# url-kaist/UV-SLAM

Hardware: AMD Instinct MI355X
Metric: sliding-window solves/sec (10 KF, 150 pts, 40 lines, 3 VP) (higher is better)
Workload: dtype f64; 1 GPU; W10-P150-L40-V3 x 256 independent windows per GPU (BASELINE configs[2]); single window (configs[1]) in single_window, the 20k-point window (configs[3]) in large_window (both with --full); windows_per_gpu=256, frames=11, points=150, lines=40, vp_tagged_lines=30, prior=True, parallelism=replicas x1

## Files before the change

uv-slam_amd/csrc/uvs_solve_kernel.h:

```cpp
#pragma once
#include <hip/hip_runtime.h>
#include <utility>
#include "../../include/uvs_solver.h"
#include "uvs_layout.h"
#include "uvs_factors.h"

namespace uvsdev {


#ifndef UVS_X_PLAIN_TID
static __device__ __forceinline__ int lane_tid() { int t = threadIdx.x; asm volatile("" : "+v"(t)); return t; }
#else
static __device__ __forceinline__ int lane_tid() { return threadIdx.x; }
#endif
static constexpr int NT = UVS_NT;
static constexpr int NW = NT / 64;
static constexpr bool ROLES = NT > 256;
static constexpr int ET = ROLES ? 256 : NT;
static constexpr int EW = ET / 64;
static constexpr int GT0 = NT - UVS_GT;
UVS_DEV int wave_uniform() { return __builtin_amdgcn_readfirstlane((int)(threadIdx.x >> 6)); }
UVS_DEV bool role_eval() { return !ROLES || wave_uniform() < EW; }
#ifndef UVS_X_NO_LINE_ROTATE
UVS_DEV int line_lane() { return ROLES ? (lane_tid() ^ 256) : lane_tid(); }
// ... 101 lines not shown
    *sq = g; *rsq = 2.0 * hh;
}
UVS_DEV void block_reduce(double* sh, double* s , double* mx) {
    const int tid = lane_tid(), lane = tid & 63, wv = tid >> 6;
    __syncthreads();
#pragma unroll
    for (int k = 0; k < 4; ++k) { const double t = wave_sum(s[k]); if (lane == 0) sh[L_RED + wv * 5 + k] = t; }
    { const double t = wave_max(*mx); if (lane == 0) sh[L_RED + wv * 5 + 4] = t; }
    __syncthreads();
    double a[4] = {0, 0, 0, 0}, m = 0.0;
#pragma unroll
    for (int w = 0; w < NW; ++w) {
#pragma unroll
        for (int k = 0; k < 4; ++k) a[k] += sh[L_RED + w * 5 + k];
        m = fmax(m, sh[L_RED + w * 5 + 4]);
    }
#pragma unroll
    for (int k = 0; k < 4; ++k) s[k] = a[k];
    *mx = m;
}

UVS_DEV void lacc_set(double* sh, double cost, double gmax) {
    const int tid = lane_tid();
    if (tid < ET) sh[L_LCOST + tid] = cost;
    const double wm = wave_max(gmax);
    if ((tid & 63) == 0) sh[L_LGMAX + (tid >> 6)] = wm;
}
UVS_DEV void lacc_add(double* sh, double cost, double gmax) {
    const int tid = lane_tid();
    if (tid < ET) sh[L_LCOST + tid] += cost;
    const double wm = wave_max(gmax);
    if ((tid & 63) == 0) sh[L_LGMAX + (tid >> 6)] = fmax(sh[L_LGMAX + (tid >> 6)], wm);
}
UVS_DEV double lacc_cost(const double* sh) { const int tid = lane_tid(); return tid < ET ? sh[L_LCOST + tid] : 0.0; }
UVS_DEV double lacc_gmax(const double* sh) { return sh[L_LGMAX + (lane_tid() >> 6)]; }

struct Ctx {
    const DevWin* hdr;
    const double* bd;
    const int* bi;
    double* ws;
    double* sh;
    KOpts o;
    int ltrig_ok = 0;
    int ptab_ok = 0;
};

UVS_DEV const double* line_trig_of(const Ctx& c, const double* line) {
    const DevWin& h = *c.hdr;
    if (!c.ltrig_ok) return nullptr;
    return line == c.ws + h.w_line0 ? c.ws + h.w_ltrig0 : (line == c.ws + h.w_line1 ? c.ws + h.w_ltrig1 : nullptr);
}

UVS_DEV void stage_rotations(const Ctx& c, const double* x) {
    const int tid = lane_tid();
    if (tid < UVS_NF) quat_to_R(x + 7 * tid + 3, c.sh + L_RF + 9 * tid);
    else if (tid == UVS_NF) { quat_to_R(x + 176 + 3, c.sh + L_EX); c.sh[L_EX + 9] = x[176]; c.sh[L_EX + 10] = x[177]; c.sh[L_EX + 11] = x[178]; }
    else if (tid == UVS_RELO_FRAME && c.hdr->relo_on) quat_to_R(x + 184 + 3, c.sh + L_RF + 9 * UVS_RELO_FRAME);
}
UVS_DEV const double* pose_of(const double* x, int f) { return x + (f > UVS_NF ? 184 : 7 * f); }

UVS_DEV void load_point_obs(const Ctx& c, int o, double td, double* pi, double* pj, double* vij) {
    const DevWin& h = *c.hdr;
    const double* m = c.bd + h.d_ptmeas + o; const int st = h.pt_stride;
    pi[0] = m[0]; pi[1] = m[st]; pi[2] = m[2 * st]; pj[0] = m[3 * st]; pj[1] = m[4 * st]; pj[2] = m[5 * st];
    if (h.td_on) {
        const double* v = c.bd + h.d_ptvel + o;
        vij[0] = v[0]; vij[1] = v[st]; vij[2] = v[2 * st]; vij[3] = v[3 * st];
        const double di = td - v[4 * st], dj = td - v[5 * st];
        pi[0] -= di * vij[0]; pi[1] -= di * vij[1]; pj[0] -= dj * vij[2]; pj[1] -= dj * vij[3];
    }
}

UVS_DEV void stage_prior_tables(const Ctx& c) {
    const int tid = lane_tid();
    const DevWin& h = *c.hdr;
    if (h.prior_n <= 0) return;
    int* tab = (int*)(c.sh + L_PTAB);
    if (tid < 4 * UVS_MAX_PRIOR_BLOCKS) tab[tid] = c.bi[h.i_prior + tid];
    if (tid < 9 * UVS_MAX_PRIOR_BLOCKS) c.sh[L_PX0 + tid] = c.bd[h.d_prior + h.prior_n * h.prior_n + 2 * h.prior_n + tid];
}
UVS_DEV void prior_dx(const Ctx& c, const double* x) {
    const int tid = lane_tid() - 64;
    const DevWin& h = *c.hdr;
    if (h.prior_n > 0 && tid >= 0 && tid < h.prior_nb) {
        int kind, frame, size, idx;
        double x0[9];
        if (c.ptab_ok) {
            const int* tab = (const int*)(c.sh + L_PTAB);
            kind = tab[tid]; frame = tab[16 + tid]; size = tab[32 + tid]; idx = tab[48 + tid];
#pragma unroll
            for (int k = 0; k < 9; ++k) x0[k] = c.sh[L_PX0 + 9 * tid + k];
        } else {
            const int* pt = c.bi + h.i_prior;
            kind = pt[tid]; frame = pt[16 + tid]; size = pt[32 + tid]; idx = pt[48 + tid];
            const double* x0g = c.bd + h.d_prior + h.prior_n * h.prior_n + 2 * h.prior_n + 9 * tid;
#pragma unroll
            for (int k = 0; k < 9; ++k) x0[k] = x0g[k];
        }
        const double* xb = (kind == UVS_BLOCK_POSE) ? x + 7 * frame : (kind == UVS_BLOCK_SPEEDBIAS) ? x + 77 + 9 * frame : (kind == UVS_BLOCK_TD) ? x + 183 : x + 176;
        double* dx = c.sh + L_PDX + idx;
        if (size != 7) { for (int k = 0; k < size; ++k) dx[k] = xb[k] - x0[k]; }
        else {
            dx[0] = xb[0] - x0[0]; dx[1] = xb[1] - x0[1]; dx[2] = xb[2] - x0[2];
            double qi[4], e[4]; quat_inv(x0 + 3, qi); quat_mul(qi, xb + 3, e);
            const double sg = (e[3] >= 0.0) ? 2.0 : -2.0;
            dx[3] = sg * e[0]; dx[4] = sg * e[1]; dx[5] = sg * e[2];
        }
    }
}
UVS_DEV double prior_quad(const Ctx& c, int dst = L_PR) {
    const DevWin& h = *c.hdr;
    const int n = h.prior_n, tid = lane_tid();
    double cost = 0.0;
    if (n <= 0) return cost;
    const double* H0 = c.ws + h.w_prior_h0;
    const int parts = (NT / n) < 4 ? (NT / n) : 4;
    const int part = tid / n, row = tid - part * n;
    const double g0v = tid < n ? c.ws[h.w_prior_h0 + UVS_PH_G0(n) + tid] : 0.0, c0v = tid == 0 ? c.ws[h.w_prior_h0 + UVS_PH_C0(n)] : 0.0;
    if (part < parts) {
        const int kb = (n * part) / parts, ke = (n * (part + 1)) / parts;
        double p8[8] = {0, 0, 0, 0, 0, 0, 0, 0};
        for (int k = kb; k < ke; k += PR_UN) {
            double jv[PR_UN];
#pragma unroll
            for (int u = 0; u < PR_UN; ++u) jv[u] = H0[(k + u < ke ? k + u : kb) * n + row];
#pragma unroll
            for (int u = 0; u < PR_UN; ++u) if (k + u < ke) p8[u & 7] += jv[u] * c.sh[L_PDX + k + u];
        }
        c.sh[L_S + 128 * part + row] = ((p8[0] + p8[1]) + (p8[2] + p8[3])) + ((p8[4] + p8[5]) + (p8[6] + p8[7]));
    }
    __syncthreads();
    if (tid < n) {
        double y = c.sh[L_S + tid];
        for (int p = 1; p < parts; ++p) y += c.sh[L_S + 128 * p + tid];
        c.sh[dst + tid] = y;
        cost = c.sh[L_PDX + tid] * (g0v + 0.5 * y);
        if (tid == 0) cost += c0v;
    }
    return cost;
}
UVS_DEV double prior_cost_share(const Ctx& c, int src) {
    const DevWin& h = *c.hdr;
    const int n = h.prior_n, tid = lane_tid();
    double cost = 0.0;
    if (tid < n) {
        cost = c.sh[L_PDX + tid] * (c.ws[h.w_prior_h0 + UVS_PH_G0(n) + tid] + 0.5 * c.sh[src + tid]);
        if (tid == 0) cost += c.ws[h.w_prior_h0 + UVS_PH_C0(n)];
    }
    return cost;
}
UVS_DEV double prior_residual_rows(const Ctx& c) {
    const DevWin& h = *c.hdr;
    const int n = h.prior_n, tid = lane_tid();
    double cost = 0.0;
    if (tid < n) {
        const double* Jr = c.bd + h.d_prior + (size_t)tid * n;
        double s = c.bd[h.d_prior + n * n + tid];
        for (int k = 0; k < n; ++k) s += Jr[k] * c.sh[L_PDX + k];
        c.sh[L_PR + tid] = s;
        cost = 0.5 * s * s;
    }
    return cost;
}

UVS_DEV void cost_imu_raw(const Ctx& c, const double* x, int lane0) {
    const DevWin& h = *c.hdr;
    const int b = lane_tid() - lane0;
    double* rs = c.sh + L_S + 1024;
    if (b >= 0 && b < h.n_imu) {
        const int fi = c.bi[h.i_imu + 2 * b], skip = c.bi[h.i_imu + 2 * b + 1];
        if (!skip) {
            const double* blk = c.bd + h.d_imu + (size_t)b * UVS_IMU_STRIDE;
            double r[15];
            imu_raw(blk, blk + UVS_IMU_JAC, c.o.G, x + 7 * fi, x + 77 + 9 * fi, x + 7 * (fi + 1), x + 77 + 9 * (fi + 1), r, nullptr);
#pragma unroll
            for (int i = 0; i < 15; ++i) rs[16 * b + i] = r[i];
        }
    }
}
template <int PB = CP_PB, int LB = CP_LB>
UVS_DEV double cost_pass(const Ctx& c, const double* x, const double* invd, const double* line, int po0, int po1, int lo0, int lo1, bool with_imu) {
    const DevWin& h = *c.hdr;
    const int tid = lane_tid();
    const double* RF = c.sh + L_RF; const double* ric = c.sh + L_EX; const double* tic = c.sh + L_EX + 9;
    const double* ltrig = line_trig_of(c, line);
    double cost = 0.0;
    long long tq_ = clock64();
#define UVS_CQ(slot) if (c.o.debug == 1 && tid == 0) { const long long t_ = clock64(); c.sh[L_WPROF + slot] += (double)(t_ - tq_); tq_ = t_; }
    const int imu_lane0 = ROLES ? NT - 64 : 0;
#ifndef UVS_X_NO_IMU_WAVE
    if (ROLES && with_imu) cost_imu_raw(c, x, imu_lane0);
#endif
    for (int o0 = po0 + tid; o0 < po1; o0 += PB * NT) {
        int lm[PB], fi[PB], fj[PB]; bool in[PB];
        double pi[PB][3], pj[PB][3], vij[PB][4], idp[PB];
#pragma unroll
        for (int u = 0; u < PB; ++u) {
            const int o = o0 + u * NT; in[u] = o < po1;
            const int oo = in[u] ? o : o0;
            lm[u] = c.bi[h.i_pt_lm + oo]; fi[u] = c.bi[h.i_pt_fi + oo]; fj[u] = c.bi[h.i_pt_fj + oo];
            load_point_obs(c, oo, x[183], pi[u], pj[u], vij[u]);
        }
#pragma unroll
        for (int u = 0; u < PB; ++u) idp[u] = invd[lm[u]];
#pragma unroll
        for (int u = 0; u < PB; ++u) {
            if (!in[u]) continue;
            double r[2];
            point_eval<false, false>(x + 7 * fi[u], RF + 9 * fi[u], pose_of(x, fj[u]), RF + 9 * fj[u], ric, tic, idp[u], pi[u], pj[u], c.o.sqrt_info, r, nullptr, nullptr, nullptr, nullptr);
            double sc; cost += 0.5 * cauchy(c.o.loss_pt, r[0] * r[0] + r[1] * r[1], &sc);
        }
    }
    for (int o0 = lo0 + UVS_COST_LINE_LANE; o0 < lo1; o0 += LB * NT) {
        int lm[LB], fj[LB], hv[LB]; bool in[LB];
        double ms[LB][9], lp[LB][4] = {}, tg[LB][8];
        const int st = h.ln_stride;
#pragma unroll
        for (int u = 0; u < LB; ++u) {
            const int o = o0 + u * NT; in[u] = o < lo1;
            const int oo = in[u] ? o : o0;
            lm[u] = c.bi[h.i_ln_lm + oo]; fj[u] = c.bi[h.i_ln_fj + oo]; hv[u] = c.bi[h.i_ln_vp + oo];
            const double* m = c.bd + h.d_lnmeas + oo;
#pragma unroll
            for (int q = 0; q < 9; ++q) ms[u][q] = m[q * st];
        }
#pragma unroll
        for (int u = 0; u < LB; ++u) {
            if (ltrig) {
#pragma unroll
                for (int q = 0; q < 8; ++q) tg[u][q] = ltrig[8 * lm[u] + q];
            } else {
#pragma unroll
                for (int q = 0; q < 4; ++q) lp[u][q] = line[4 * lm[u] + q];
            }
        }
#pragma unroll
        for (int u = 0; u < LB; ++u) {
            if (!in[u]) continue;
            const double sp[3] = {ms[u][0], ms[u][1], ms[u][2]}, ep[3] = {ms[u][3], ms[u][4], ms[u][5]}, vp[3] = {ms[u][6], ms[u][7], ms[u][8]};
            LineGeom g;
            line_geom<false>(x + 7 * fj[u], x + 7 * fj[u] + 3, RF + 9 * fj[u], ric, tic, lp[u], g, ltrig ? tg[u] : nullptr);
            double r[2], sc;
            line_residual<false>(g, sp, ep, c.o.line_factor, r, nullptr, nullptr);
            cost += 0.5 * cauchy(c.o.loss_ln, r[0] * r[0] + r[1] * r[1], &sc);
            if (hv[u]) { double rv; vp_residual<false>(g, vp, c.o.vp_factor, &rv, nullptr, nullptr); cost += 0.5 * cauchy(c.o.loss_vp, rv * rv, &sc); }
        }
    }
    UVS_CQ(2)
    if (with_imu) {
        double* rs = c.sh + L_S + 1024;
#ifndef UVS_X_NO_IMU_WAVE
        if (!ROLES)
#endif
        cost_imu_raw(c, x, 0);
        __syncthreads();
        const int b = tid >> 4, i = tid & 15;
        if (b < h.n_imu && i < 15 && !c.bi[h.i_imu + 2 * b + 1]) {
            const double* W = c.ws + h.w_imu_w + (size_t)b * UVS_IMU_WS + i * 15;
            double wv[15];
#pragma unroll
            for (int k = 0; k < 15; ++k) wv[k] = (k >= i) ? W[k] : 0.0;
            double sacc = 0.0;
#pragma unroll
            for (int k = 0; k < 15; ++k) sacc += wv[k] * rs[16 * b + k];
            cost += 0.5 * sacc * sacc;
        }
    }
    UVS_CQ(3)
    return cost;
}

typedef double d4_t __attribute__((ext_vector_type(4)));

UVS_DEV double* sblk(double* sh, int i, int j) { return sh + L_S + (((i * (i + 1)) >> 1) + j) * UVS_BLK_SZ; }

UVS_DEV double rcp_newton(double x) {
    double y = __builtin_amdgcn_rcp(x);
    double e = fma(-x, y, 1.0); y = fma(y, e, y);
    e = fma(-x, y, 1.0); y = fma(y, e, y);
    return y;
}

struct MiniCtx { double* sh; struct { int debug; } o; };
template <bool TR = false>
UVS_DEV void chol_update_item(double* sh, int i, int cc, int j0, int j1, int lane, d4_t& acc) {
    const int li = lane & 15, lk = lane >> 4;
    const bool rhs = (i == UVS_NF);
    const double* Bj = sblk(sh, cc, j0) + li * UVS_BLK_LD + lk;
    const double* Ai = rhs ? sh + L_DLT + 16 * j0 + lk : sblk(sh, i, j0) + li * UVS_BLK_LD + lk;
    const int astep = rhs ? 16 : UVS_BLK_SZ;
    if (j0 >= j1) return;
    double a0[4], b0[4], a1[4], b1[4];
#define UVS_CH_LOAD(AV, BV) { _Pragma("unroll") for (int q = 0; q < 4; ++q) { AV[q] = Ai[4 * q]; BV[q] = Bj[4 * q]; } Bj += UVS_BLK_SZ; Ai += astep; }
#define UVS_CH_MFMA(AV, BV) { _Pragma("unroll") for (int q = 0; q < 4; ++q) acc = TR ? __builtin_amdgcn_mfma_f64_16x16x4f64(BV[q], AV[q], acc, 0, 0, 1) : __builtin_amdgcn_mfma_f64_16x16x4f64(AV[q], BV[q], acc, 0, 0, 1); }
    UVS_CH_LOAD(a0, b0)
    for (int j = j0;;) {
        if (j + 1 < j1) UVS_CH_LOAD(a1, b1)
        UVS_CH_MFMA(a0, b0)
        if (++j >= j1) break;
        if (j + 1 < j1) UVS_CH_LOAD(a0, b0)
        UVS_CH_MFMA(a1, b1)
        if (++j >= j1) break;
    }
// ... 1843 lines not shown
        asm_imu(c, N);
    }
#ifndef UVS_X_NO_PRIOR_AHEAD
    asm_prior_add(c, pa);
#else
    asm_prior(c);
#endif
    __syncthreads();
    UVS_TLOG(c, 26);
    asm_finish(c, x, first && !redamp, radius, lacc_cost(c.sh) + ic, lacc_gmax(c.sh), 0);
    UVS_TLOG(c, 27);
}

UVS_DEV void linearize(const Ctx& c, const double* x, const double* invd, const double* line, bool first, double radius, int prep_mode, GAcc& A) {
    if (ROLES) { linearize_roles(c, x, invd, line, first, radius, prep_mode, false); return; }
    const DevWin& h = *c.hdr;
    const int grp = gather_group(c);
    gacc_zero(A);
    { const double pc = lin_prep(c, x, prep_mode); lacc_set(c.sh, pc, 0.0); }
    {
        ChunkDesc d = chunk_desc(c, 0);
        for (int ch = 0; ch < h.n_chunks; ++ch) {
            chunk_eval(c, d, x, invd, line, first, radius);
            chunk_gather(c, d, grp, A);
            if (ch + 1 < h.n_chunks) d = chunk_desc(c, ch + 1);
        }
    }
    ImuN N;
    const double ic = lin_imu(c, x, N);
    lin_assemble(c, x, first, radius, grp, A, N, lacc_cost(c.sh) + ic, lacc_gmax(c.sh));
}

UVS_DEV void relinearize_damping(const Ctx& c, const double* x, double radius, GAcc& A) {
    if (ROLES) { linearize_roles(c, x, nullptr, nullptr, false, radius, 2, true); return; }
    const DevWin& h = *c.hdr;
    const int grp = gather_group(c);
    (void)lin_prep(c, x, 2);
    {
        ChunkDesc d = chunk_desc(c, 0);
        for (int ch = 0; ch < h.n_chunks; ++ch) {
            redamp_prep(c, d, radius);
            redamp_gather(c, d, grp, A);
            if (ch + 1 < h.n_chunks) d = chunk_desc(c, ch + 1);
        }
    }
    ImuN N;
    const double ic = lin_imu(c, x, N);
    lin_assemble(c, x, false, radius, grp, A, N, lacc_cost(c.sh) + ic, lacc_gmax(c.sh));
}

#ifndef UVS_BS_FRAME_LANE0
#define UVS_BS_FRAME_LANE0 192
#endif
template <int LNBT = BS_LNB, int PSB = 4, bool STREAM = false>
UVS_DEV void backsub_candidate(const Ctx& c, const double* invd, const double* line, double* invd_c, double* line_c,
                                  int pk0, int pk1, int lk0, int lk1, bool with_frames, double* sums_out, double* lstep = nullptr) {
    const DevWin& h = *c.hdr;
    double* sh = c.sh;
    const int tid = lane_tid();
    const double* d = sh + L_DLT;
    double gd = 0.0, dd2 = 0.0, step2 = 0.0, xc2 = 0.0;
    const bool td_on = h.td_on != 0;
    const bool ex_on = h.ex_on != 0, relo_on = h.relo_on != 0;
    double* ltrig_c = const_cast<double*>(line_trig_of(c, line_c));
    const bool relo2 = h.relo2 != 0;
    if (relo2) relo2_backsub(c);
    else if (relo_on) {
        if (tid < 6) sh[L_DLT + 16 * UVS_RELO_FRAME + tid] = d[UVS_EX_INDEX(tid)];
        __syncthreads();
    }
    if (with_frames && tid < UVS_RD && ((tid & 15) < 15 || (td_on && tid == UVS_TD_INDEX) || ((ex_on | relo_on) && tid < 96))) { gd += sh[L_G + tid] * d[tid]; dd2 += sh[L_DD + tid] * d[tid] * d[tid]; }
    const int ft = tid - UVS_BS_FRAME_LANE0;
    if (with_frames && ft >= 0 && ft < UVS_NF) {
        double xp[7];
        pose_plus(sh + L_X + 7 * ft, d + 16 * ft, xp);
#pragma unroll
        for (int k = 0; k < 7; ++k) { sh[L_XC + 7 * ft + k] = xp[k]; const double e = xp[k] - sh[L_X + 7 * ft + k]; step2 += e * e; xc2 += xp[k] * xp[k]; }
#pragma unroll
        for (int k = 0; k < 9; ++k) { const double v = sh[L_X + 77 + 9 * ft + k] + d[16 * ft + 6 + k]; sh[L_XC + 77 + 9 * ft + k] = v; step2 += d[16 * ft + 6 + k] * d[16 * ft + 6 + k]; xc2 += v * v; }
    }
    if (with_frames && ft == UVS_NF) {
        if (ex_on) {
            double de[6], xp[7];
#pragma unroll
            for (int k = 0; k < 6; ++k) de[k] = d[UVS_EX_INDEX(k)];
            pose_plus(sh + L_X + 176, de, xp);
#pragma unroll
            for (int k = 0; k < 7; ++k) { sh[L_XC + 176 + k] = xp[k]; const double e = xp[k] - sh[L_X + 176 + k]; step2 += e * e; xc2 += xp[k] * xp[k]; }
        } else for (int k = 0; k < 7; ++k) sh[L_XC + 176 + k] = sh[L_X + 176 + k];
        const double dtd = td_on ? d[UVS_TD_INDEX] : 0.0, tdc = sh[L_X + 183] + dtd;
        sh[L_XC + 183] = tdc;
        if (td_on) { step2 += dtd * dtd; xc2 += tdc * tdc; }
        if (relo_on) {
            double de[6], xp[7];
#pragma unroll
            for (int k = 0; k < 6; ++k) de[k] = d[16 * UVS_RELO_FRAME + k];
            if (relo2) {
                const double* W = c.ws + h.w_relo2;
#pragma unroll
                for (int k = 0; k < 6; ++k) { gd -= W[R2_G + k] * W[R2_MG + k]; dd2 += W[R2_DD + k] * de[k] * de[k]; }
            }
            pose_plus(sh + L_X + 184, de, xp);
#pragma unroll
            for (int k = 0; k < 7; ++k) { sh[L_XC + 184 + k] = xp[k]; const double e = xp[k] - sh[L_X + 184 + k]; step2 += e * e; xc2 += xp[k] * xp[k]; }
        } else for (int k = 0; k < 7; ++k) sh[L_XC + 184 + k] = sh[L_X + 184 + k];
    }
    const int* pbeg = c.bi + h.i_pt_beg;
    for (int k = pk0 + tid; k < pk1; k += NT) {
        const int b0 = pbeg[k], b1 = pbeg[k + 1];
        const double* px = c.ws + h.w_pt_x + 4 * (size_t)k;
        const double* Eg = c.ws + h.w_pt_E + 6 * (size_t)(b0 + h.pt_xslots * k);
        double px0 = 0.0, px1 = 0.0, px2 = 0.0, iv0 = 0.0;
        if (STREAM) { px0 = px[0]; px1 = px[1]; px2 = px[2]; iv0 = invd[k]; }
        double t = 0.0;
        if (b1 > b0) {
            const int ns = b1 - b0 + 1;
            for (int s0 = 0; s0 < ns; s0 += PSB) {
                int fr[PSB]; double ev[PSB][6];
#pragma unroll
                for (int u = 0; u < PSB; ++u) {
                    const int sl = s0 + u, slc = sl < ns ? sl : 0;
                    fr[u] = slc == 0 ? c.bi[h.i_pt_fi + b0] : c.bi[h.i_pt_fj + b0 + slc - 1];
#pragma unroll
                    for (int a = 0; a < 6; ++a) ev[u][a] = Eg[6 * slc + a];
                }
#pragma unroll
                for (int u = 0; u < PSB; ++u) {
                    if (s0 + u >= ns) continue;
#pragma unroll
                    for (int a = 0; a < 6; ++a) t += ev[u][a] * d[16 * fr[u] + a];
                }
            }
            if (td_on) t += Eg[6 * (b1 - b0 + 1)] * d[UVS_TD_INDEX];
            if (ex_on) {
                const double* e = Eg + 6 * (b1 - b0 + 1 + (td_on ? 1 : 0));
#pragma unroll
                for (int a = 0; a < 6; ++a) t += e[a] * d[UVS_EX_INDEX(a)];
            }
        }
        if (!STREAM) { px0 = px[0]; px1 = px[1]; px2 = px[2]; iv0 = invd[k]; }
        const double dl = -px0 - t;
        const double v = iv0 + dl;
        invd_c[k] = v;
        if (lstep) lstep[k] = dl;
        gd += px1 * (dl + t); dd2 += px2 * dl * dl; step2 += dl * dl; xc2 += v * v;
    }
    constexpr int LNB = LNBT;
    const int* lbeg = c.bi + h.i_ln_beg;
#ifndef UVS_X_NO_LINE_QSPLIT
    if ((ROLES && ltrig_c) || STREAM) {
        for (int e = 4 * lk0 + line_lane(); e < 4 * lk1; e += NT) {
            const int k = e >> 2, q = e & 3;
            const int b0 = lbeg[k], b1 = lbeg[k + 1];
            const double* lx = c.ws + h.w_ln_x + UVS_LN_X * (size_t)k;
            double t = 0.0;
            constexpr int QB = STREAM ? 8 : 4;
            const double lxq = STREAM ? lx[q] : 0.0, lx4 = STREAM ? lx[4 + q] : 0.0, lx8 = STREAM ? lx[8 + q] : 0.0, ln0 = STREAM ? line[4 * k + q] : 0.0;
            for (int o = b0; o < b1; o += QB) {
                int fr[QB]; double yv[QB][6];
#pragma unroll
                for (int u = 0; u < QB; ++u) {
                    const int oc = o + u < b1 ? o + u : o;
                    fr[u] = c.bi[h.i_ln_fj + oc];
                    const double* Y = c.ws + h.w_ln_Y + 24 * (size_t)oc + 6 * q;
#pragma unroll
                    for (int a = 0; a < 6; ++a) yv[u][a] = Y[a];
                }
#pragma unroll
                for (int u = 0; u < QB; ++u) {
                    if (o + u >= b1) continue;
#pragma unroll
                    for (int a = 0; a < 6; ++a) t += yv[u][a] * d[16 * fr[u] + a];
                }
            }
            const double dl = -(STREAM ? lxq : lx[q]) - t;
            const double v = (STREAM ? ln0 : line[4 * k + q]) + dl;
            line_c[4 * k + q] = v;
            if (lstep) lstep[h.n_points + 4 * k + q] = dl;
            gd += (STREAM ? lx4 : lx[4 + q]) * (dl + t); dd2 += (STREAM ? lx8 : lx[8 + q]) * dl * dl; step2 += dl * dl; xc2 += v * v;
            if (ltrig_c) sincos(v, ltrig_c + 8 * k + 2 * q, ltrig_c + 8 * k + 2 * q + 1);
        }
    } else
#endif
    for (int k = lk0 + line_lane(); k < lk1; k += NT) {
        const int b0 = lbeg[k], b1 = lbeg[k + 1];
        const double* lx = c.ws + h.w_ln_x + UVS_LN_X * (size_t)k;
        double t[4] = {0.0, 0.0, 0.0, 0.0};
        for (int o = b0; o < b1; o += LNB) {
            int fr[LNB]; double yv[LNB][24];
#pragma unroll
            for (int u = 0; u < LNB; ++u) {
                const int oc = o + u < b1 ? o + u : o;
                fr[u] = c.bi[h.i_ln_fj + oc];
                const double* Y = c.ws + h.w_ln_Y + 24 * (size_t)oc;
#pragma unroll
                for (int q = 0; q < 24; ++q) yv[u][q] = Y[q];
            }
#pragma unroll
            for (int u = 0; u < LNB; ++u) {
                if (o + u >= b1) continue;
#pragma unroll
                for (int q = 0; q < 4; ++q)
#pragma unroll
                    for (int a = 0; a < 6; ++a) t[q] += yv[u][6 * q + a] * d[16 * fr[u] + a];
            }
        }
        double vn[4];
#pragma unroll
        for (int q = 0; q < 4; ++q) {
            const double dl = -lx[q] - t[q];
            const double v = line[4 * k + q] + dl;
            line_c[4 * k + q] = v; vn[q] = v;
            if (lstep) lstep[h.n_points + 4 * k + q] = dl;
            gd += lx[4 + q] * (dl + t[q]); dd2 += lx[8 + q] * dl * dl; step2 += dl * dl; xc2 += v * v;
        }
        if (ltrig_c) line_trig(vn, ltrig_c + 8 * k);
    }
    double s4[4] = {gd, dd2, step2, xc2};
    double mx = 0.0;
    block_reduce(sh, s4, &mx);
    if (tid == 0) {
        sh[L_CTRL + C_MCC] = 0.5 * (s4[1] - s4[0]);
        sh[L_CTRL + C_STEP2] = s4[2];
        sh[L_CTRL + C_XC2] = s4[3];
        if (sums_out) { sums_out[0] = s4[0]; sums_out[1] = s4[1]; sums_out[2] = s4[2]; sums_out[3] = s4[3]; }
    }
    __syncthreads();
}

UVS_DEV double ambient_sqnorm(const Ctx& c, const double* x, const double* invd, const double* line) {
    const DevWin& h = *c.hdr;
    const int tid = lane_tid();
    double s = 0.0;
    if (tid < 176) s += x[tid] * x[tid];
    if (tid == 183 && h.td_on) s += x[183] * x[183];
    if (tid >= 176 && tid < 183 && h.ex_on) s += x[tid] * x[tid];
    if (tid >= 184 && tid < 191 && h.relo_on) s += x[tid] * x[tid];
    for (int k = tid; k < h.n_points; k += NT) s += invd[k] * invd[k];
    for (int k = tid; k < 4 * h.n_lines; k += NT) s += line[k] * line[k];
    double s4[4] = {s, 0, 0, 0}, mx = 0.0;
    block_reduce(c.sh, s4, &mx);
    return s4[0];
}

UVS_DEV void imu_whiten_block(const double* cov, double* W, double* scr , int lane) {
    double m[15];
#pragma unroll
    for (int i = 0; i < 15; ++i) m[i] = lane < 15 ? cov[i * 15 + lane] : (i == lane - 15 ? 1.0 : 0.0);
#pragma unroll
    for (int k = 0; k < 15; ++k) {
        int piv = k; double best = fabs(bcast_lane(m[k], k));
#pragma unroll
        for (int i = k + 1; i < 15; ++i) { const double v = fabs(bcast_lane(m[i], k)); if (v > best) { best = v; piv = i; } }
        piv = __builtin_amdgcn_readfirstlane(piv);
#pragma unroll
        for (int i = k + 1; i < 15; ++i) if (piv == i) { const double t = m[k]; m[k] = m[i]; m[i] = t; }
        const double dinv = 1.0 / bcast_lane(m[k], k);
#pragma unroll
        for (int i = k + 1; i < 15; ++i) {
            const double f = bcast_lane(m[i], k) * dinv;
            if (lane >= k) m[i] -= f * m[k];
        }
    }
#pragma unroll
    for (int k = 14; k >= 0; --k) {
        const double dinv = 1.0 / bcast_lane(m[k], k);
        m[k] *= dinv;
#pragma unroll
        for (int i = 0; i < k; ++i) {
            const double f = bcast_lane(m[i], k);
            m[i] -= f * m[k];
        }
    }
    if (lane >= 15 && lane < 30) {
#pragma unroll
        for (int i = 0; i < 15; ++i) scr[i * 15 + (lane - 15)] = m[i];
    }
    wave_sync();
    double a[15], Lr[15];
#pragma unroll
// ... 61 lines not shown
            const double* Ja = Jl + (ca < n ? ca : 0); const double* Jb = Jl + (cb < n ? cb : 0);
            d4_t acc = {0.0, 0.0, 0.0, 0.0};
            for (int k0 = 0; k0 < n; k0 += 20) {
                double av[5], bv[5];
#pragma unroll
                for (int u = 0; u < 5; ++u) {
                    const int i = k0 + 4 * u + lk, ic = i < n ? i : n - 1;
                    const double a = Ja[ic * n], bq = Jb[ic * n];
                    av[u] = (ca < n && i < n) ? a : 0.0; bv[u] = (cb < n && i < n) ? bq : 0.0;
                }
#pragma unroll
                for (int u = 0; u < 5; ++u) acc = __builtin_amdgcn_mfma_f64_16x16x4f64(av[u], bv[u], acc, 0, 0, 0);
            }
#pragma unroll
            for (int q = 0; q < 4; ++q) {
                const int ra = 16 * ta + lk + 4 * q;
                if (ra < n && cb < n) { H0[ra * n + cb] = acc[q]; if (ta != tb) H0[cb * n + ra] = acc[q]; }
            }
        }
        if (tid < n) {
            double p4[4] = {0, 0, 0, 0};
            for (int i = 0; i < n; ++i) p4[i & 3] += Jl[i * n + tid] * r0l[i];
            H0[UVS_PH_G0(n) + tid] = (p4[0] + p4[1]) + (p4[2] + p4[3]);
        }
        if (tid == NT - 1) { double s2 = 0.0; for (int i = 0; i < n; ++i) s2 += r0l[i] * r0l[i]; H0[UVS_PH_C0(n)] = 0.5 * s2; }
        if (tid < UVS_RD) {
            const int a = inv[tid];
            double v = 0.0;
            if (a >= 0) for (int i = 0; i < n; ++i) v += Jl[i * n + a] * Jl[i * n + a];
            H0[UVS_PH_HD(n) + tid] = v;
        }
        __threadfence_block();
    }
}

struct DebugOut {
    double* S;
    double* g;
    double* hd;
    double* dd;
    double* step;
    double* scal;
};

#define UVS_DSTEP_FR (UVS_RD + 24)
struct DebugStep {
    const double* radii;
    int n;
    long long stride;
    double* steps;
    double* scal;
};

template <bool DSTEP>
UVS_DEV void k_solve_body(char* blobs, const long long* blob_off, double* ws_all, const long long* ws_off,
                          KOpts o, uvs_report* reports, DebugOut dbg, DebugStep ds, double* sh) {
    const int tid = lane_tid(), wdx = blockIdx.x;
    char* blob = blobs + blob_off[wdx];
    Ctx c;
    c.hdr = (const DevWin*)blob; c.bd = (const double*)blob; c.bi = (const int*)blob; c.ws = ws_all + ws_off[wdx]; c.sh = sh; c.o = o;
    const DevWin& h = *c.hdr;
    uvs_report* rep = reports + wdx;
    if (tid < UVS_XDIM) sh[L_X + tid] = c.bd[h.d_frames + tid];
    for (int k = tid; k < h.n_points; k += NT) c.ws[h.w_invd0 + k] = c.bd[h.d_invd + k];
    for (int k = tid; k < 4 * h.n_lines; k += NT) c.ws[h.w_line0 + k] = c.bd[h.d_line + k];
    for (int k = tid; k < h.n_lines; k += NT) line_trig(c.bd + h.d_line + 4 * k, c.ws + h.w_ltrig0 + 8 * k);
    c.ltrig_ok = 1;
#ifndef UVS_X_NO_PTAB
    stage_prior_tables(c); c.ptab_ok = 1;
#endif
    for (int i = tid; i < (int)(sizeof(uvs_report) / 4); i += NT) ((int*)rep)[i] = 0;
    if (tid < 24) sh[L_PROF + tid] = (tid == 23) ? (double)clock64() : 0.0;
    if (tid < 8) sh[L_WPROF + tid] = 0.0;
    setup_window(c, (double*)blob);
    __syncthreads();
    UVS_PROF(c, P_SETUP);
    int cur = 0;
    double* invd[2] = {c.ws + h.w_invd0, c.ws + h.w_invd1};
    double* line[2] = {c.ws + h.w_line0, c.ws + h.w_line1};
    double radius = o.r0, decr = 2.0;
    double cost = 0.0, gmax = 0.0, x_norm = 0.0;
    int it = 0, invalid = 0, nsucc = 0, term = UVS_TERM_NO_CONVERGENCE, status = UVS_OK;
    bool need_lin = true, first = true;
    GAcc gacc;
    int prep_mode = 0;
    int pending = 0;
    const long long t_wall0 = wall_clock64();
    while (true) {
        if (it >= o.max_it && !first) { term = UVS_TERM_NO_CONVERGENCE; break; }
        if (o.max_ticks > 0 && !first) {
            __syncthreads();
            if (tid == 0) sh[L_CTRL + C_TIMEUP] = (wall_clock64() - t_wall0 >= o.max_ticks) ? 1.0 : 0.0;
            __syncthreads();
            if (sh[L_CTRL + C_TIMEUP] != 0.0) { term = UVS_TERM_MAX_TIME; break; }
        }
        if (need_lin) {
#ifndef UVS_X_NO_REDAMP
            if (prep_mode == 2 && !first && h.redamp_ok && o.redamp) relinearize_damping(c, sh + L_X, radius, gacc);
            else
#endif
            linearize(c, sh + L_X, invd[cur], line[cur], first, radius, prep_mode, gacc);
            need_lin = false;
            const double lc = sh[L_CTRL + C_COST];
            gmax = sh[L_CTRL + C_GMAX];
            if (first) {
                const double xn2 = ambient_sqnorm(c, sh + L_X, invd[0], line[0]);
                x_norm = sqrt(xn2); cost = lc; first = false;
                if (tid == 0) { rep->initial_cost = cost; rep->cost[0] = cost; rep->radius[0] = radius; rep->gradient_max_norm[0] = gmax; rep->accepted[0] = 1; }
                if (!isfinite(cost)) { term = UVS_TERM_NUMERIC_FAILURE; status = UVS_ERR_NUMERIC; break; }
            } else if (pending > 0) {
                cost = lc;
                if (tid == 0) { rep->cost[pending] = cost; rep->gradient_max_norm[pending] = gmax; }
            }
            pending = 0;
        }
        if (it >= o.max_it) { term = UVS_TERM_NO_CONVERGENCE; break; }
        if (gmax <= o.gtol) { term = UVS_TERM_GRADIENT_TOL; break; }
        if (radius <= o.rmin) { term = UVS_TERM_MIN_RADIUS; break; }
        ++it;
        const int ti = it < UVS_MAX_ITER ? it : UVS_MAX_ITER;
        if (tid < UVS_RD) sh[L_DLT + tid] = -sh[L_G + tid];
        if (o.debug && it == 1 && dbg.S) {
            __syncthreads();
            for (int t = tid; t < UVS_RD * UVS_RD; t += NT) { const int i = t / UVS_RD, j = t - i * UVS_RD; dbg.S[t] = (j <= i) ? sh[L_S + sidx(i, j)] : 0.0; }
            if (tid < UVS_RD) { dbg.g[tid] = sh[L_G + tid]; dbg.hd[tid] = sh[L_HD + tid]; dbg.dd[tid] = sh[L_DD + tid]; }
        }
        UVS_PROF(c, P_MISC);
        UVS_TLOG(c, 30);
        chol_factor(c);
        UVS_PROF(c, P_CHOL);
        UVS_TLOG(c, 31);
        chol_solve(c);
        UVS_PROF(c, P_TRSV);
        UVS_TLOG(c, 32);
        bool ok = sh[L_CTRL + C_CHOLOK] != 0.0;
        backsub_candidate(c, invd[cur], line[cur], invd[cur ^ 1], line[cur ^ 1], 0, h.n_points, 0, h.n_lines, true, nullptr,
                          DSTEP ? ds.steps + (size_t)(it - 1) * ds.stride + UVS_DSTEP_FR : nullptr);
        UVS_PROF(c, P_BACKSUB);
        UVS_TLOG(c, 33);
        const double mcc = sh[L_CTRL + C_MCC], step2 = sh[L_CTRL + C_STEP2], xc2 = sh[L_CTRL + C_XC2];
        if (DSTEP) {
            if (tid < UVS_DSTEP_FR) ds.steps[(size_t)(it - 1) * ds.stride + tid] = sh[L_DLT + tid];
            if (tid == 0) { double* sc = ds.scal + (size_t)(it - 1) * UVS_DEBUG_SCAL_LEN; sc[0] = cost; sc[1] = gmax; sc[2] = ok ? 1.0 : 0.0; sc[3] = mcc; sc[4] = step2; }
            if (it >= ds.n) break;
            radius = ds.radii[it]; need_lin = true; prep_mode = 2;
            __syncthreads();
            continue;
        }
        if (o.debug && it == 1 && dbg.S) {
            if (tid < UVS_RD) dbg.step[tid] = sh[L_DLT + tid];
            if (tid == 0) { dbg.scal[0] = cost; dbg.scal[1] = gmax; dbg.scal[2] = ok ? 1.0 : 0.0; dbg.scal[3] = mcc; dbg.scal[4] = step2; }
        }
        if (!isfinite(mcc) || !isfinite(step2)) ok = false;
        if (tid == 0) rep->model_cost_change[ti] = mcc;
        if (!ok || !(mcc > 0.0)) {
            ++invalid;
            radius = radius / decr; decr *= 2.0; need_lin = true; prep_mode = 2;
            if (tid == 0) { rep->accepted[ti] = -1; rep->cost[ti] = cost; rep->candidate_cost[ti] = cost; rep->radius[ti] = radius; rep->gradient_max_norm[ti] = gmax; }
            if (invalid >= o.max_invalid) { term = UVS_TERM_INVALID_STEPS; break; }
            continue;
        }
        invalid = 0;
        __syncthreads();
        long long tc_ = clock64();
        stage_rotations(c, sh + L_XC);
        prior_dx(c, sh + L_XC);
        __syncthreads();
        if (o.debug == 1 && tid == 0) { const long long t_ = clock64(); sh[L_WPROF + 0] += (double)(t_ - tc_); tc_ = t_; }
        UVS_TLOG(c, 34);
        double cc_ = prior_quad(c, L_PRC);
        UVS_TLOG(c, 35);
        if (o.debug == 1 && tid == 0) { const long long t_ = clock64(); sh[L_WPROF + 1] += (double)(t_ - tc_); tc_ = t_; }
        cc_ += cost_pass(c, sh + L_XC, invd[cur ^ 1], line[cur ^ 1], 0, h.n_pt_obs, 0, h.n_ln_obs, true);
        UVS_TLOG(c, 36);
        double s4[4] = {cc_, 0, 0, 0}, mx = 0.0;
        block_reduce(sh, s4, &mx);
        UVS_TLOG(c, 37);
        UVS_PROF(c, P_COST);
        double cand = s4[0];
        if (!isfinite(cand)) cand = 1.7976931348623157e308;
        const double step_norm = sqrt(step2);
        const double rel = (cost - cand) / mcc;
        const bool successful = rel > o.min_rel;
        if (tid == 0) { rep->candidate_cost[ti] = cand; rep->step_norm[ti] = step_norm; rep->relative_decrease[ti] = rel; rep->cost[ti] = cost; rep->radius[ti] = radius; rep->gradient_max_norm[ti] = gmax; }
        bool stop = false;
        if (step_norm <= o.ptol * (x_norm + o.ptol)) { term = UVS_TERM_PARAMETER_TOL; stop = true; }
        else if (fabs(cost - cand) <= o.ftol * cost) { term = UVS_TERM_FUNCTION_TOL; stop = true; }
        if (stop && !(o.keep_cand && successful)) break;
        if (successful) {
            __syncthreads();
            if (tid < UVS_XDIM) sh[L_X + tid] = sh[L_XC + tid];
            cur ^= 1; ++nsucc;
            x_norm = sqrt(xc2);
            { const double t3 = 2.0 * rel - 1.0; radius = radius / fmax(1.0 / 3.0, 1.0 - t3 * t3 * t3); }
            radius = fmin(o.rmax, radius);
            decr = 2.0;
            cost = cand;
            need_lin = true; pending = ti; prep_mode = 1;
            if (tid == 0) { rep->accepted[ti] = 1; rep->cost[ti] = cost; rep->radius[ti] = radius; }
            if (stop) break;
        } else {
            radius = radius / decr; decr *= 2.0; need_lin = true; prep_mode = 2;
            if (tid == 0) { rep->accepted[ti] = 0; rep->radius[ti] = radius; }
        }
    }
    __syncthreads();
    UVS_PROF(c, P_MISC);
    if (o.debug && dbg.scal && tid < P_LAST) dbg.scal[8 + tid] = sh[L_PROF + tid];
    if (o.debug && dbg.scal && tid < 8) dbg.scal[24 + tid] = sh[L_WPROF + tid];
    if (tid < UVS_XDIM) c.ws[h.w_out + tid] = sh[L_X + tid];
    for (int k = tid; k < h.n_points; k += NT) c.ws[h.w_out + UVS_XDIM + k] = invd[cur][k];
    for (int k = tid; k < 4 * h.n_lines; k += NT) c.ws[h.w_out + UVS_XDIM + h.n_points + k] = line[cur][k];
    if (h.out_host) {
        double* od = (double*)h.out_host;
        if (tid < UVS_XDIM) od[tid] = sh[L_X + tid];
        for (int k = tid; k < h.n_points; k += NT) od[UVS_XDIM + k] = invd[cur][k];
        for (int k = tid; k < 4 * h.n_lines; k += NT) od[UVS_XDIM + h.n_points + k] = line[cur][k];
    }
    if (tid == 0) {
        rep->status = status; rep->termination = term; rep->num_iterations = it; rep->num_successful = nsucc; rep->final_cost = cost;
        ((DevWin*)blob)->cur_sel = cur;
    }
}
#ifndef UVS_DSTEP_ONLY
__global__ __launch_bounds__(NT) void k_solve(char* blobs, const long long* blob_off, double* ws_all, const long long* ws_off,
                                              KOpts o, uvs_report* reports, DebugOut dbg) {
// ... 68 lines not shown
```

Measured before the change: 183,100 solves/s.

## Overlap candidate rotation, prior and IMU cost staging with back-substitution

Result: slower. 179,500 solves/s (-2.0%).

```diff
diff --git a/uv-slam_amd/csrc/uvs_solve_kernel.h b/uv-slam_amd/csrc/uvs_solve_kernel.h
--- a/uv-slam_amd/csrc/uvs_solve_kernel.h
+++ b/uv-slam_amd/csrc/uvs_solve_kernel.h
@@ -177,8 +177,9 @@
     return line == c.ws + h.w_line0 ? c.ws + h.w_ltrig0 : (line == c.ws + h.w_line1 ? c.ws + h.w_ltrig1 : nullptr);
 }
 
-UVS_DEV void stage_rotations(const Ctx& c, const double* x) {
-    const int tid = lane_tid();
+UVS_DEV void stage_rotations(const Ctx& c, const double* x, int lane0 = 0) {
+    const int tid = lane_tid() - lane0;
+    if (tid < 0) return;
     if (tid < UVS_NF) quat_to_R(x + 7 * tid + 3, c.sh + L_RF + 9 * tid);
     else if (tid == UVS_NF) { quat_to_R(x + 176 + 3, c.sh + L_EX); c.sh[L_EX + 9] = x[176]; c.sh[L_EX + 10] = x[177]; c.sh[L_EX + 11] = x[178]; }
     else if (tid == UVS_RELO_FRAME && c.hdr->relo_on) quat_to_R(x + 184 + 3, c.sh + L_RF + 9 * UVS_RELO_FRAME);
@@ -205,8 +206,8 @@
     if (tid < 4 * UVS_MAX_PRIOR_BLOCKS) tab[tid] = c.bi[h.i_prior + tid];
     if (tid < 9 * UVS_MAX_PRIOR_BLOCKS) c.sh[L_PX0 + tid] = c.bd[h.d_prior + h.prior_n * h.prior_n + 2 * h.prior_n + tid];
 }
-UVS_DEV void prior_dx(const Ctx& c, const double* x) {
-    const int tid = lane_tid() - 64;
+UVS_DEV void prior_dx(const Ctx& c, const double* x, int lane0 = 64) {
+    const int tid = lane_tid() - lane0;
     const DevWin& h = *c.hdr;
     if (h.prior_n > 0 && tid >= 0 && tid < h.prior_nb) {
         int kind, frame, size, idx;
@@ -234,28 +235,21 @@
         }
     }
 }
-UVS_DEV double prior_quad(const Ctx& c, int dst = L_PR) {
-    const DevWin& h = *c.hdr;
-    const int n = h.prior_n, tid = lane_tid();
+UVS_DEV void prior_quad_item(const Ctx& c, const double* H0, int n, int parts, int part, int row) {
+    const int kb = (n * part) / parts, ke = (n * (part + 1)) / parts;
+    double p8[8] = {0, 0, 0, 0, 0, 0, 0, 0};
+    for (int k = kb; k < ke; k += PR_UN) {
+        double jv[PR_UN];
+#pragma unroll
+        for (int u = 0; u < PR_UN; ++u) jv[u] = H0[(k + u < ke ? k + u : kb) * n + row];
+#pragma unroll
+        for (int u = 0; u < PR_UN; ++u) if (k + u < ke) p8[u & 7] += jv[u] * c.sh[L_PDX + k + u];
+    }
+    c.sh[L_S + 128 * part + row] = ((p8[0] + p8[1]) + (p8[2] + p8[3])) + ((p8[4] + p8[5]) + (p8[6] + p8[7]));
+}
+UVS_DEV double prior_quad_finish(const Ctx& c, int n, int parts, int dst, double g0v, double c0v) {
+    const int tid = lane_tid();
     double cost = 0.0;
-    if (n <= 0) return cost;
-    const double* H0 = c.ws + h.w_prior_h0;
-    const int parts = (NT / n) < 4 ? (NT / n) : 4;
-    const int part = tid / n, row = tid - part * n;
-    const double g0v = tid < n ? c.ws[h.w_prior_h0 + UVS_PH_G0(n) + tid] : 0.0, c0v = tid == 0 ? c.ws[h.w_prior_h0 + UVS_PH_C0(n)] : 0.0;
-    if (part < parts) {
-        const int kb = (n * part) / parts, ke = (n * (part + 1)) / parts;
-        double p8[8] = {0, 0, 0, 0, 0, 0, 0, 0};
-        for (int k = kb; k < ke; k += PR_UN) {
-            double jv[PR_UN];
-#pragma unroll
-            for (int u = 0; u < PR_UN; ++u) jv[u] = H0[(k + u < ke ? k + u : kb) * n + row];
-#pragma unroll
-            for (int u = 0; u < PR_UN; ++u) if (k + u < ke) p8[u & 7] += jv[u] * c.sh[L_PDX + k + u];
-        }
-        c.sh[L_S + 128 * part + row] = ((p8[0] + p8[1]) + (p8[2] + p8[3])) + ((p8[4] + p8[5]) + (p8[6] + p8[7]));
-    }
-    __syncthreads();
     if (tid < n) {
         double y = c.sh[L_S + tid];
         for (int p = 1; p < parts; ++p) y += c.sh[L_S + 128 * p + tid];
@@ -264,6 +258,20 @@
         if (tid == 0) cost += c0v;
     }
     return cost;
+}
+UVS_DEV int prior_quad_parts(int n) { return (NT / n) < 4 ? (NT / n) : 4; }
+UVS_DEV double prior_quad(const Ctx& c, int dst = L_PR) {
+    const DevWin& h = *c.hdr;
+    const int n = h.prior_n, tid = lane_tid();
+    double cost = 0.0;
+    if (n <= 0) return cost;
+    const double* H0 = c.ws + h.w_prior_h0;
+    const int parts = prior_quad_parts(n);
+    const int part = tid / n, row = tid - part * n;
+    const double g0v = tid < n ? c.ws[h.w_prior_h0 + UVS_PH_G0(n) + tid] : 0.0, c0v = tid == 0 ? c.ws[h.w_prior_h0 + UVS_PH_C0(n)] : 0.0;
+    if (part < parts) prior_quad_item(c, H0, n, parts, part, row);
+    __syncthreads();
+    return prior_quad_finish(c, n, parts, dst, g0v, c0v);
 }
 UVS_DEV double prior_cost_share(const Ctx& c, int src) {
     const DevWin& h = *c.hdr;
@@ -289,10 +297,11 @@
     return cost;
 }
 
+static constexpr int IMU_RS = 1024, IMU_SW = IMU_RS + 16 * UVS_NF;
 UVS_DEV void cost_imu_raw(const Ctx& c, const double* x, int lane0) {
     const DevWin& h = *c.hdr;
     const int b = lane_tid() - lane0;
-    double* rs = c.sh + L_S + 1024;
+    double* rs = c.sh + L_S + IMU_RS;
     if (b >= 0 && b < h.n_imu) {
         const int fi = c.bi[h.i_imu + 2 * b], skip = c.bi[h.i_imu + 2 * b + 1];
         if (!skip) {
@@ -304,10 +313,28 @@
         }
     }
 }
-template <int PB = CP_PB, int LB = CP_LB>
-UVS_DEV double cost_pass(const Ctx& c, const double* x, const double* invd, const double* line, int po0, int po1, int lo0, int lo1, bool with_imu) {
+UVS_DEV void cost_imu_whiten_wave(const Ctx& c, int lane0) {
+    const DevWin& h = *c.hdr;
+    const double* rs = c.sh + L_S + IMU_RS;
+    for (int it = lane_tid() - lane0; it < 16 * h.n_imu; it += 64) {
+        const int b = it >> 4, i = it & 15;
+        double sacc = 0.0;
+        if (i < 15 && !c.bi[h.i_imu + 2 * b + 1]) {
+            const double* W = c.ws + h.w_imu_w + (size_t)b * UVS_IMU_WS + i * 15;
+            double wv[15];
+#pragma unroll
+            for (int k = 0; k < 15; ++k) wv[k] = (k >= i) ? W[k] : 0.0;
+#pragma unroll
+            for (int k = 0; k < 15; ++k) sacc += wv[k] * rs[16 * b + k];
+        }
+        c.sh[L_S + IMU_SW + it] = sacc;
+    }
+}
+template <int PB = CP_PB, int LB = CP_LB, bool PICK = false>
+UVS_DEV double cost_pass(const Ctx& c, const double* x, const double* invd, const double* line, int po0, int po1, int lo0, int lo1, bool with_imu, bool imu_done = false) {
     const DevWin& h = *c.hdr;
     const int tid = lane_tid();
+    const bool picked = PICK && imu_done;
     const double* RF = c.sh + L_RF; const double* ric = c.sh + L_EX; const double* tic = c.sh + L_EX + 9;
     const double* ltrig = line_trig_of(c, line);
     double cost = 0.0;
@@ -315,7 +342,7 @@
 #define UVS_CQ(slot) if (c.o.debug == 1 && tid == 0) { const long long t_ = clock64(); c.sh[L_WPROF + slot] += (double)(t_ - tq_); tq_ = t_; }
     const int imu_lane0 = ROLES ? NT - 64 : 0;
 #ifndef UVS_X_NO_IMU_WAVE
-    if (ROLES && with_imu) cost_imu_raw(c, x, imu_lane0);
+    if (ROLES && with_imu && !picked) cost_imu_raw(c, x, imu_lane0);
 #endif
     for (int o0 = po0 + tid; o0 < po1; o0 += PB * NT) {
         int lm[PB], fi[PB], fj[PB]; bool in[PB];
@@ -373,8 +400,13 @@
         }
     }
     UVS_CQ(2)
-    if (with_imu) {
-        double* rs = c.sh + L_S + 1024;
+    if (picked) {
+        if ((tid >> 4) < h.n_imu) {
+            const double sacc = c.sh[L_S + IMU_SW + tid];
+            cost += 0.5 * sacc * sacc;
+        }
+    } else if (with_imu) {
+        double* rs = c.sh + L_S + IMU_RS;
 #ifndef UVS_X_NO_IMU_WAVE
         if (!ROLES)
 #endif
@@ -2324,9 +2356,11 @@
 #ifndef UVS_BS_FRAME_LANE0
 #define UVS_BS_FRAME_LANE0 192
 #endif
-template <int LNBT = BS_LNB, int PSB = 4, bool STREAM = false>
-UVS_DEV void backsub_candidate(const Ctx& c, const double* invd, const double* line, double* invd_c, double* line_c,
-                                  int pk0, int pk1, int lk0, int lk1, bool with_frames, double* sums_out, double* lstep = nullptr) {
+template <int LNBT = BS_LNB, int PSB = 4, bool STREAM = false, bool EARLY = false, bool OVERLAP = false>
+UVS_DEV bool backsub_candidate(const Ctx& c, const double* invd, const double* line, double* invd_c, double* line_c,
+                                  int pk0, int pk1, int lk0, int lk1, bool with_frames, double* sums_out, double* lstep = nullptr, double* prior_gc = nullptr) {
+    static_assert(!OVERLAP || (ROLES && (UVS_BS_FRAME_LANE0 & 63) == 0 && UVS_BS_FRAME_LANE0 / 64 != NW - 1), "OVERLAP: the frame lanes open a wave of their own, the last wave carries the IMU blocks");
+    constexpr bool SCAL_EARLY = STREAM || EARLY;
     const DevWin& h = *c.hdr;
     double* sh = c.sh;
     const int tid = lane_tid();
@@ -2378,12 +2412,46 @@
         } else for (int k = 0; k < 7; ++k) sh[L_XC + 184 + k] = sh[L_X + 184 + k];
     }
     const int* pbeg = c.bi + h.i_pt_beg;
+    const bool overlap = OVERLAP && with_frames && !relo_on && !relo2;
+    const int kp0 = pk0 + tid, ep0 = 4 * lk0 + line_lane();
+    int pf_pb0 = 0, pf_pb1 = 0, pf_lb0 = 0, pf_lb1 = 0;
+    double pf_p[4] = {0.0, 0.0, 0.0, 0.0}, pf_l[4] = {0.0, 0.0, 0.0, 0.0};
+    if (OVERLAP && overlap) {
+        if (kp0 < pk1) { const double* px = c.ws + h.w_pt_x + 4 * (size_t)kp0; pf_pb0 = pbeg[kp0]; pf_pb1 = pbeg[kp0 + 1]; pf_p[0] = px[0]; pf_p[1] = px[1]; pf_p[2] = px[2]; pf_p[3] = invd[kp0]; }
+        if (ep0 < 4 * lk1) {
+            const int k = ep0 >> 2, q = ep0 & 3; const double* lx = c.ws + h.w_ln_x + UVS_LN_X * (size_t)k;
+            pf_lb0 = c.bi[h.i_ln_beg + k]; pf_lb1 = c.bi[h.i_ln_beg + k + 1]; pf_l[0] = lx[q]; pf_l[1] = lx[4 + q]; pf_l[2] = lx[8 + q]; pf_l[3] = line[4 * k + q];
+        }
+        if (prior_gc && h.prior_n > 0) { prior_gc[0] = tid < h.prior_n ? c.ws[h.w_prior_h0 + UVS_PH_G0(h.prior_n) + tid] : 0.0; prior_gc[1] = tid == 0 ? c.ws[h.w_prior_h0 + UVS_PH_C0(h.prior_n)] : 0.0; }
+        const int wv = wave_uniform();
+        if (wv == UVS_BS_FRAME_LANE0 / 64) {
+            wave_sync();
+            stage_rotations(c, sh + L_XC, UVS_BS_FRAME_LANE0);
+            prior_dx(c, sh + L_XC, UVS_BS_FRAME_LANE0 + 16);
+            UVS_TLOG(c, 34);
+        }
+        __syncthreads();
+        if (wv == UVS_BS_FRAME_LANE0 / 64 && h.prior_n > 0) {
+            const int n = h.prior_n, parts = prior_quad_parts(n);
+            const double* H0 = c.ws + h.w_prior_h0;
+            for (int it = tid - UVS_BS_FRAME_LANE0; it < parts * n; it += 64) { const int part = it / n; prior_quad_item(c, H0, n, parts, part, it - part * n); }
+            UVS_TLOG(c, 35);
+        }
+        if (wv == NW - 1) {
+            cost_imu_raw(c, sh + L_XC, NT - 64);
+            wave_sync();
+            cost_imu_whiten_wave(c, NT - 64);
+            UVS_TLOG(c, 38);
+        }
+    }
     for (int k = pk0 + tid; k < pk1; k += NT) {
-        const int b0 = pbeg[k], b1 = pbeg[k + 1];
+        const bool pf = OVERLAP && overlap && k == kp0;
+        const int b0 = pf ? pf_pb0 : pbeg[k], b1 = pf ? pf_pb1 : pbeg[k + 1];
         const double* px = c.ws + h.w_pt_x + 4 * (size_t)k;
         const double* Eg = c.ws + h.w_pt_E + 6 * (size_t)(b0 + h.pt_xslots * k);
         double px0 = 0.0, px1 = 0.0, px2 = 0.0, iv0 = 0.0;
-        if (STREAM) { px0 = px[0]; px1 = px[1]; px2 = px[2]; iv0 = invd[k]; }
+        if (pf) { px0 = pf_p[0]; px1 = pf_p[1]; px2 = pf_p[2]; iv0 = pf_p[3]; }
+        else if (SCAL_EARLY) { px0 = px[0]; px1 = px[1]; px2 = px[2]; iv0 = invd[k]; }
         double t = 0.0;
         if (b1 > b0) {
             const int ns = b1 - b0 + 1;
@@ -2410,7 +2478,7 @@
                 for (int a = 0; a < 6; ++a) t += e[a] * d[UVS_EX_INDEX(a)];
             }
         }
-        if (!STREAM) { px0 = px[0]; px1 = px[1]; px2 = px[2]; iv0 = invd[k]; }
+        if (!SCAL_EARLY && !pf) { px0 = px[0]; px1 = px[1]; px2 = px[2]; iv0 = invd[k]; }
         const double dl = -px0 - t;
         const double v = iv0 + dl;
         invd_c[k] = v;
@@ -2423,11 +2491,13 @@
     if ((ROLES && ltrig_c) || STREAM) {
         for (int e = 4 * lk0 + line_lane(); e < 4 * lk1; e += NT) {
             const int k = e >> 2, q = e & 3;
-            const int b0 = lbeg[k], b1 = lbeg[k + 1];
+            const bool pf = OVERLAP && overlap && e == ep0;
+            const int b0 = pf ? pf_lb0 : lbeg[k], b1 = pf ? pf_lb1 : lbeg[k + 1];
             const double* lx = c.ws + h.w_ln_x + UVS_LN_X * (size_t)k;
             double t = 0.0;
-            constexpr int QB = STREAM ? 8 : 4;
-            const double lxq = STREAM ? lx[q] : 0.0, lx4 = STREAM ? lx[4 + q] : 0.0, lx8 = STREAM ? lx[8 + q] : 0.0, ln0 = STREAM ? line[4 * k + q] : 0.0;
+            constexpr int QB = SCAL_EARLY ? 8 : 4;
+            const bool have = SCAL_EARLY || pf;
+            const double lxq = pf ? pf_l[0] : SCAL_EARLY ? lx[q] : 0.0, lx4 = pf ? pf_l[1] : SCAL_EARLY ? lx[4 + q] : 0.0, lx8 = pf ? pf_l[2] : SCAL_EARLY ? lx[8 + q] : 0.0, ln0 = pf ? pf_l[3] : SCAL_EARLY ? line[4 * k + q] : 0.0;
             for (int o = b0; o < b1; o += QB) {
                 int fr[QB]; double yv[QB][6];
 #pragma unroll
@@ -2445,11 +2515,11 @@
                     for (int a = 0; a < 6; ++a) t += yv[u][a] * d[16 * fr[u] + a];
                 }
             }
-            const double dl = -(STREAM ? lxq : lx[q]) - t;
-            const double v = (STREAM ? ln0 : line[4 * k + q]) + dl;
+            const double dl = -(have ? lxq : lx[q]) - t;
+            const double v = (have ? ln0 : line[4 * k + q]) + dl;
             line_c[4 * k + q] = v;
             if (lstep) lstep[h.n_points + 4 * k + q] = dl;
-            gd += (STREAM ? lx4 : lx[4 + q]) * (dl + t); dd2 += (STREAM ? lx8 : lx[8 + q]) * dl * dl; step2 += dl * dl; xc2 += v * v;
+            gd += (have ? lx4 : lx[4 + q]) * (dl + t); dd2 += (have ? lx8 : lx[8 + q]) * dl * dl; step2 += dl * dl; xc2 += v * v;
             if (ltrig_c) sincos(v, ltrig_c + 8 * k + 2 * q, ltrig_c + 8 * k + 2 * q + 1);
         }
     } else
@@ -2498,6 +2568,7 @@
         if (sums_out) { sums_out[0] = s4[0]; sums_out[1] = s4[1]; sums_out[2] = s4[2]; sums_out[3] = s4[3]; }
     }
     __syncthreads();
+    return overlap;
 }
 
 UVS_DEV double ambient_sqnorm(const Ctx& c, const double* x, const double* invd, const double* line) {
@@ -2665,6 +2736,16 @@
     double* scal;
 };
 
+#ifndef UVS_X_NO_BS_TWO_TRIPS
+static constexpr bool CAND_TWO_TRIPS = ROLES;
+#else
+static constexpr bool CAND_TWO_TRIPS = false;
+#endif
+#ifndef UVS_X_NO_CAND_OVERLAP
+static constexpr bool CAND_OVERLAP = ROLES;
+#else
+static constexpr bool CAND_OVERLAP = false;
+#endif
 template <bool DSTEP>
 UVS_DEV void k_solve_body(char* blobs, const long long* blob_off, double* ws_all, const long long* ws_off,
                           KOpts o, uvs_report* reports, DebugOut dbg, DebugStep ds, double* sh) {
@@ -2747,8 +2828,9 @@
         UVS_PROF(c, P_TRSV);
         UVS_TLOG(c, 32);
         bool ok = sh[L_CTRL + C_CHOLOK] != 0.0;
-        backsub_candidate(c, invd[cur], line[cur], invd[cur ^ 1], line[cur ^ 1], 0, h.n_points, 0, h.n_lines, true, nullptr,
-                          DSTEP ? ds.steps + (size_t)(it - 1) * ds.stride + UVS_DSTEP_FR : nullptr);
+        double prior_gc[2] = {0.0, 0.0};
+        const bool overlapped = backsub_candidate<BS_LNB, CAND_TWO_TRIPS ? 8 : 4, false, CAND_TWO_TRIPS, CAND_OVERLAP>(c, invd[cur], line[cur], invd[cur ^ 1], line[cur ^ 1], 0, h.n_points, 0, h.n_lines, true, nullptr,
+                          DSTEP ? ds.steps + (size_t)(it - 1) * ds.stride + UVS_DSTEP_FR : nullptr, prior_gc);
         UVS_PROF(c, P_BACKSUB);
         UVS_TLOG(c, 33);
         const double mcc = sh[L_CTRL + C_MCC], step2 = sh[L_CTRL + C_STEP2], xc2 = sh[L_CTRL + C_XC2];
@@ -2774,17 +2856,22 @@
             continue;
         }
         invalid = 0;
-        __syncthreads();
         long long tc_ = clock64();
-        stage_rotations(c, sh + L_XC);
-        prior_dx(c, sh + L_XC);
-        __syncthreads();
-        if (o.debug == 1 && tid == 0) { const long long t_ = clock64(); sh[L_WPROF + 0] += (double)(t_ - tc_); tc_ = t_; }
-        UVS_TLOG(c, 34);
-        double cc_ = prior_quad(c, L_PRC);
-        UVS_TLOG(c, 35);
+        double cc_;
+        if (CAND_OVERLAP && overlapped) {
+            cc_ = h.prior_n > 0 ? prior_quad_finish(c, h.prior_n, prior_quad_parts(h.prior_n), L_PRC, prior_gc[0], prior_gc[1]) : 0.0;
+        } else {
+            __syncthreads();
+            stage_rotations(c, sh + L_XC);
+            prior_dx(c, sh + L_XC);
+            __syncthreads();
+            if (o.debug == 1 && tid == 0) { const long long t_ = clock64(); sh[L_WPROF + 0] += (double)(t_ - tc_); tc_ = t_; }
+            UVS_TLOG(c, 34);
+            cc_ = prior_quad(c, L_PRC);
+            UVS_TLOG(c, 35);
+        }
         if (o.debug == 1 && tid == 0) { const long long t_ = clock64(); sh[L_WPROF + 1] += (double)(t_ - tc_); tc_ = t_; }
-        cc_ += cost_pass(c, sh + L_XC, invd[cur ^ 1], line[cur ^ 1], 0, h.n_pt_obs, 0, h.n_ln_obs, true);
+        cc_ += cost_pass<CP_PB, CP_LB, CAND_OVERLAP>(c, sh + L_XC, invd[cur ^ 1], line[cur ^ 1], 0, h.n_pt_obs, 0, h.n_ln_obs, true, overlapped);
         UVS_TLOG(c, 36);
         double s4[4] = {cc_, 0, 0, 0}, mx = 0.0;
         block_reduce(sh, s4, &mx);
```
